# nipe1783/cudaSBMP

Measured on AMD Instinct MI355X. Metric: collision-checked samples/sec + time-to-first-solution, R2 car @1/2/4/8 GPUs, higher is better.
Workload: dtype f32; 1 GPU; c3: car, 262144 samples/iter/GPU, M=16777216, reference 5-box workspace, goal disabled, complete GNew clear; gnew_clear=complete, samples_per_iter_per_gpu=262144, maxTreeSize=16777216, numDisc=10, obstacles=5, seed=20240807, mean_frontier=1018, mean_accepted=1017, parallelism=single GPU

## Files before the change

cudasbmp_amd/_native.py:

```python
from __future__ import annotations

import ctypes
import os

_PKG = os.path.dirname(os.path.abspath(__file__))
LIB_PATH = os.path.join(_PKG, "libsbmp.so")

SBMP_OK = 0
SBMP_AGENT_CAR = 0
SBMP_AGENT_POINT = 1
SBMP_COMM_ID_BYTES = 128
SBMP_BATCH_REFERENCE = 0
SBMP_BATCH_FILL = 1


class NativeLibraryError(RuntimeError):
    pass


class SbmpError(RuntimeError):
    def __init__(self, status: int, func: str, msg: str):
        super().__init__(f"{func} failed with status {status}: {msg}")
        self.status = status

# ... 39 lines not shown


class ExpandBatchArgs(ctypes.Structure):
    _fields_ = [("count", ctypes.c_int), ("parents", ctypes.c_void_p), ("rng", ctypes.c_void_p),
                ("obstacles", ctypes.c_void_p), ("obstaclesCount", ctypes.c_int), ("agent", ctypes.c_int),
                ("numDisc", ctypes.c_int), ("agentLength", ctypes.c_float), ("width", ctypes.c_float),
                ("height", ctypes.c_float), ("N", ctypes.c_int), ("n", ctypes.c_int), ("R1Score", ctypes.c_void_p),
                ("R2Avail", ctypes.c_void_p), ("children", ctypes.c_void_p), ("valid", ctypes.c_void_p),
                ("r1", ctypes.c_void_p), ("r2", ctypes.c_void_p), ("accept", ctypes.c_void_p)]


class InsertBatchArgs(ctypes.Structure):
    _fields_ = [("slots", ctypes.c_int), ("gnew", ctypes.c_void_p), ("unexplored", ctypes.c_void_p),
                ("uParent", ctypes.c_void_p), ("samples", ctypes.c_void_p), ("parent", ctypes.c_void_p),
                ("costs", ctypes.c_void_p), ("treeSize", ctypes.c_int), ("maxTreeSize", ctypes.c_int),
                ("goalX", ctypes.c_float), ("goalY", ctypes.c_float), ("goalThreshold", ctypes.c_float),
                ("fixGNewClear", ctypes.c_int), ("inserted", ctypes.c_void_p), ("goalIndex", ctypes.c_void_p)]


class PathInfo(ctypes.Structure):
    _fields_ = [(n, ctypes.c_int) for n in ("stepForm", "obstacleForm", "residentGroups", "neededGroups", "exchange",
                                            "nranks", "rank", "commRanks", "listMirror",
                                            "fusedExchange", "oneshotCheck", "mirrorCheck", "fusedCheck", "rowTableLds",
                                            "rcpDivisions")]


class BatchInfo(ctypes.Structure):
    _fields_ = [(n, ctypes.c_int) for n in ("count", "groupsPerMember", "residentGroups", "membersPerLaunch",
                                            "launchesPerIteration", "batched")]


class GoalQuery(ctypes.Structure):
    _fields_ = [("x", ctypes.c_float), ("y", ctypes.c_float), ("radius", ctypes.c_float)]


class GoalAnswer(ctypes.Structure):
    _fields_ = [("count", ctypes.c_int), ("firstRow", ctypes.c_int), ("bestRow", ctypes.c_int),
                ("bestCost", ctypes.c_float), ("nearestRow", ctypes.c_int), ("nearestDistance", ctypes.c_float)]


class TreeRecheck(ctypes.Structure):
    _fields_ = [(n, ctypes.c_int) for n in ("rows", "alive", "blocked", "stale", "orphan", "cut", "firstDead")]


class TreeRecheckArgs(ctypes.Structure):
    _fields_ = [("state", ctypes.c_void_p), ("ctrl", ctypes.c_void_p), ("parent", ctypes.c_void_p),
                ("rows", ctypes.c_int), ("depthBound", ctypes.c_int), ("agent", ctypes.c_int),
# ... 157 lines not shown
```

cudasbmp_amd/csrc/kgmt_batch.cpp:

```cpp
#include <algorithm>
#include <cstdlib>
#include <cstring>

#include "kgmt_planner.h"

namespace sbmp {

template <typename F>
static auto for_member(int i, F f) {
    try {
        return f();
    } catch (const Error& e) {
        throw Error(e.status, "member " + std::to_string(i) + ": " + e.what());
    }
}

int BatchGroup::pack(const int* groupsPerMember, int count, int residentGroups, int* launchOfMember) {
    int launches = 0, used = 0;
    bool open = false;
    for (int i = 0; i < count; ++i) {
        const int g = groupsPerMember[i];
        if (g > residentGroups) {
            launchOfMember[i] = -1;
            open = false;
// ... 60 lines not shown
    for (int m = 0; m < B; ++m) members_[m]->begin(initials + 7 * m, goals + 7 * m, d_obstacles, nObs, seeds[m]);
    bool step = true;
    for (KgmtPlanner* k : members_) step = step && k->d_.stepMode && k->d_.hostPoll;
    for (KgmtPlanner* k : members_)
        if ((k->d_.stepMode != 0) != (members_[0]->d_.stepMode != 0))
            throw Error(SBMP_ERR_STATE, "batch members chose different forms");
    residentGroups_ = 0;
    membersPerLaunch_ = 1;
    std::fill(launchOf_.begin(), launchOf_.end(), -1);
    int nLaunches = 0;
    if (step) {
        KgmtPlanner& k0 = *members_[0];
        residentGroups_ = step_batch_resident_groups(k0.d_, k0.p_.agent, k0.expandVariant_);
        if (const char* v = getenv("SBMP_BATCH_MAX_GROUPS")) {
            const int cap = atoi(v);
            if (cap >= 0 && cap < residentGroups_) residentGroups_ = cap;
        }
        std::vector<int> groups(B);
        for (int m = 0; m < B; ++m) groups[m] = 1 + members_[m]->d_.nBlocks;
        nLaunches = pack(groups.data(), B, residentGroups_, launchOf_.data());
        if (nLaunches == 0 || std::count(launchOf_.begin(), launchOf_.end(), -1) > 0) {
            for (KgmtPlanner* k : members_) {
                k->d_.stepMode = 0;
                k->flushed_ = true;
                launch_finish(k->d_, 0, 0, stream_, k->timing(KgmtPlanner::K_FINISH));
            }
            SBMP_HIP(hipGetLastError());
            step = false;
            nLaunches = 0;
        }
    }
    batched_ = step;
    bool same = (int)launches_.size() == nLaunches;
    if (same) {
        std::vector<int> cnt(nLaunches, 0);
        for (int m = 0; m < B && batched_; ++m) cnt[launchOf_[m]]++;
        for (int l = 0; l < nLaunches; ++l) same = same && launches_[l].members == cnt[l];
    }
    if (!same) {
        SBMP_HIP(hipStreamSynchronize(stream_));
        free_launches();
        launches_.resize(nLaunches);
        for (int m = 0; m < B && batched_; ++m) {
            Launch& l = launches_[launchOf_[m]];
            if (l.members == 0) l.first = m;
            l.members++;
// ... 29 lines not shown
        launch_step_batch(k0.d_, t, expand, k0.p_.agent, k0.expandVariant_, l.dTable, l.members, l.maxGroups, stream_,
                          expand ? timer_.take(0, members_[0]->p_.profileKernels != 0) : KernelTiming());
    }
}

void BatchGroup::stage_member(KgmtPlanner* k, int t) {
    if (k->d_.stepMode) {
        k->stage_step(t);
    } else {
        k->stage_expand(t);
        k->stage_finish(t);
    }
}

void BatchGroup::enqueue(int iterations) {
    if (!begun_) throw Error(SBMP_ERR_STATE, "begin() has not been called");
    for (int i = 0; i < iterations; ++i) {
        int t = 0;
        for (KgmtPlanner* k : members_) t = k->take_iteration();
        if (t == 0) break;
        if (batched_) {
            for (KgmtPlanner* k : members_) k->upload_dev();
            issue(t, 1);
            for (KgmtPlanner* k : members_) k->flushed_ = false;
        } else {
            for (KgmtPlanner* k : members_) stage_member(k, t);
        }
        for (KgmtPlanner* k : members_) k->stage_fold(t);
    }
    SBMP_HIP(hipGetLastError());
}

void BatchGroup::flush() {
    if (!begun_) return;
    if (batched_) {
        bool any = false;
        for (KgmtPlanner* k : members_) any = any || !k->flushed_;
        if (!any) return;
        for (KgmtPlanner* k : members_) k->upload_dev();
        issue(members_[0]->t_next_, 0);
        for (KgmtPlanner* k : members_) k->flushed_ = true;
    } else {
        for (KgmtPlanner* k : members_) k->flush();
    }
}

void BatchGroup::sync() {
// ... 58 lines not shown
```

cudasbmp_amd/csrc/kgmt_device.h:

```cpp
#pragma once

#include <hip/hip_runtime.h>
#include <stdint.h>

#include <type_traits>

#include "sbmp/collision.h"
#include "sbmp/grid.h"
#include "sbmp/obstacle_grid.h"
#include "sbmp/sbmp_math.h"
#include "sbmp/xorwow.h"

#if defined(__clang__)
#pragma clang fp contract(off)
#endif

namespace sbmp {

constexpr int kBlock = 256;
constexpr int kWave = 64;
constexpr int kNoGoal = 0x7fffffff;
constexpr int kN = 16;
constexpr int kMaxR1 = kN * kN;
constexpr int kMaxR2Words = 2048;
// ... 44 lines not shown
constexpr int kNewReps = 8;
constexpr int kMaxStepBlocks = 1024;
constexpr int kNoGoalIdx = 0x7fffffff;
constexpr int kFastDivMax = 1 << 24;
constexpr int kStepEntry = 3;
constexpr int kPlannerInsertMax = 1024;
static_assert(kBlock / kWave == 4 && kMaxR1 == kBlock, "the flush and prefix code assumes 4 waves and 256 R1 cells");
constexpr int kInsertBase = 8;
constexpr int kRecordF4 = 3;

constexpr int kFxReplicas = 8;
constexpr int kFxShards = 8;
constexpr int kFxCounters = kFxReplicas * kFxShards;
constexpr int kFxStride = 32;
struct OneshotCompact {
    int nR1, rowOff, rowWords, cntOff, owned, nBlocks, newOff, newWords;
    int c16Off;
    int cR, cB, cN, total;
};

struct KgmtDev {
    int M, nSlots, nWords, nBlocks, numIterations, numDisc, N, n, nR1, nR2, nObs, cap, fixGNewClear;
    int batchRule;
    int nranks, rank;
    float width, height, agentLength, invAgentLength, goalThreshold, R1Size, R2Size, goalX, goalY;
    float rcpR1Size, rcpR2Size, rcpNumDisc, rcpAgentLength;
    float reachStep;
    float4* treeState;
    float4* treeCtrl;
    int* treeParent;
    float4* uState;
    float4* uCtrl;
    uint4* rngA;
    uint2* rngB;
    unsigned long long* gnewOut;
    unsigned long long* gnewIn;
    int* blockCountOut;
    const int* blockCountIn;
    int* pfxOut;
    const int* pfxIn;
    int* totOut;
    const int* totIn;
    unsigned long long* deltaOut;
    const unsigned long long* deltaIn;
    uint8_t* r2newOut;
    const uint8_t* r2newIn;
// ... 740 lines not shown
```

cudasbmp_amd/csrc/kgmt_kernels.hip:

```cpp
#include <hip/hip_ext.h>
#include <hip/hip_runtime.h>

#include "kgmt_device.h"
#include "kgmt_launch.h"
#include "kgmt_rules.h"

#if defined(__clang__)
#pragma clang fp contract(off)
#endif

namespace sbmp {

__device__ __forceinline__ int div_small(int a, int b) {
    int q = (int)((float)a * __builtin_amdgcn_rcpf((float)b));
    int r = a - q * b;
    if (r < 0) { --q; r += b; }
    if (r < 0) { --q; r += b; }
    if (r >= b) { ++q; r -= b; }
    if (r >= b) { ++q; }
    return q;
}

__device__ __forceinline__ int slot_div(const KgmtDev& d, int slot, int k) {
    if (k == 32) return slot >> 5;
// ... 1712 lines not shown
    int k = depth - 1;
    for (int j = node; j >= 0; j = d.treeParent[j], --k) {
        const float4 st = d.treeState[j];
        const float4 c = d.treeCtrl[j];
        rows[k] = j;
        float* o = samples + (size_t)k * 7;
        o[0] = st.x; o[1] = st.y; o[2] = st.z; o[3] = st.w;
        o[4] = c.x; o[5] = c.y; o[6] = c.z;
        costs[k] = c.w;
    }
}

__global__ void k_export_unexplored(KgmtDev d, float* samples, int* uParent) {
    for (int i = blockIdx.x * blockDim.x + threadIdx.x; i < d.nSlots; i += gridDim.x * blockDim.x) {
        const float4 s = d.uState[i];
        const float4 c = d.uCtrl[i];
        float* o = samples + (size_t)i * 7;
        o[0] = s.x; o[1] = s.y; o[2] = s.z; o[3] = s.w;
        o[4] = c.x; o[5] = c.y; o[6] = c.z;
        uParent[i] = __float_as_int(c.w);
    }
}

template <typename K, typename... Args>
static void launch(K kernel, dim3 grid, dim3 block, size_t shm, hipStream_t s, const KernelTiming& tm,
                   Args... args) {
    if (tm.start)
        hipExtLaunchKernelGGL(kernel, grid, block, (uint32_t)shm, s, tm.start, tm.stop, 0u, args...);
    else
        hipLaunchKernelGGL(kernel, grid, block, shm, s, args...);
}

int obstacle_form(const KgmtDev& d, int variant) {
    return with_obs_form(d, variant, [](auto obs) { return obs.value >= kObsReg ? kObsReg : obs.value; });
}

static size_t obs_lds_bytes(const KgmtDev& d, int obs) {
    return (obs == kObsLds || obs == kObsLds4) ? sizeof(float4) * (size_t)d.nObs : 0;
}

void launch_expand(const KgmtDev& d, int t, int agent, int blocks, int variant, hipStream_t s,
                   const KernelTiming& tm) {
    const dim3 grid(blocks), block(kBlock);
    with_obs_form(d, variant, [&](auto obs) {
        const size_t shm = obs_lds_bytes(d, obs.value);
        if (agent == 0) launch(k_expand<0, obs.value>, grid, block, shm, s, tm, d, t);
// ... 176 lines not shown

void launch_delay(double microseconds, hipStream_t s) {
    const long long ticks = (long long)(microseconds * 100.0);
    hipLaunchKernelGGL(k_delay, dim3(1), dim3(64), 0, s, ticks);
}

void launch_seed_root(const KgmtDev& d, float4 rs, float4 rc, int r1, int r2, hipStream_t s) {
    hipLaunchKernelGGL(k_seed_root, dim3(1), dim3(64), 0, s, d, rs, rc, r1, r2);
}

void launch_export_tree(const KgmtDev& d, float* samples, float* costs, hipStream_t s) {
    hipLaunchKernelGGL(k_export_tree, dim3(1024), dim3(256), 0, s, d, samples, costs);
}

void launch_solution_path(const KgmtDev& d, int node, int maxDepth, int* out, int* rows, float* samples, float* costs,
                          hipStream_t s) {
    hipLaunchKernelGGL(k_solution_path, dim3(1), dim3(64), 0, s, d, node, maxDepth, out, rows, samples, costs);
}

void launch_export_unexplored(const KgmtDev& d, float* samples, int* uParent, hipStream_t s) {
    hipLaunchKernelGGL(k_export_unexplored, dim3(1024), dim3(256), 0, s, d, samples, uParent);
}

}
```

cudasbmp_amd/csrc/kgmt_launch.h:

```cpp
#pragma once

#include <hip/hip_runtime.h>
#include <stdint.h>

#include <type_traits>
#include <vector>

#include "kgmt_device.h"

namespace sbmp {

struct KernelTiming {
    hipEvent_t start = nullptr;
    hipEvent_t stop = nullptr;
};

int obstacle_form(const KgmtDev& d, int variant);
template <int OBS>
using ObsForm = std::integral_constant<int, OBS>;

template <typename F>
auto with_obs_form(const KgmtDev& d, int variant, F f) {
    if (d.gridStart) return f(ObsForm<kObsGrid>{});
    if (d.nObs > kMaxLdsObs) return f(ObsForm<kObsGlobal>{});
// ... 56 lines not shown
    int rowOff, rows;
    int cntOff, owned, nBlocks;
    int newOff, newWords;
    int c16Off;
};
OneshotCompact oneshot_compact(const OneshotLayout& l);
void launch_oneshot(unsigned long long* const* inbox, const unsigned long long* send, unsigned long long* recv,
                    long long n, int nranks, int rank, unsigned long long seq, int* error, hipStream_t s,
                    const KernelTiming& tm = KernelTiming(), const OneshotLayout* compact = nullptr,
                    long long* tl = nullptr);
void launch_xsum(const unsigned long long* const* send, unsigned long long* const* recv, int nranks, long long n,
                 hipStream_t s);
void launch_delay(double microseconds, hipStream_t s);
void launch_fill_i32(int* p, int v, long long n, hipStream_t s);
void launch_fill_f32(float* p, float v, long long n, hipStream_t s);
void launch_init_slots(const KgmtDev& d, const Xorwow& base, const uint32_t* jumps, int nbits, int blocks,
                       hipStream_t s);
void launch_solution_path(const KgmtDev& d, int node, int maxDepth, int* out, int* rows, float* samples, float* costs,
                          hipStream_t s);
void launch_seed_root(const KgmtDev& d, float4 rs, float4 rc, int r1, int r2, hipStream_t s);
void launch_export_tree(const KgmtDev& d, float* samples, float* costs, hipStream_t s);
void launch_state_hash(const KgmtDev& d, int rows, int tp, int iters, unsigned long long* out, hipStream_t s);
void launch_export_unexplored(const KgmtDev& d, float* samples, int* uParent, hipStream_t s);

struct QueryAcc {
    unsigned long long best;
    unsigned long long nearest;
    unsigned count;
    unsigned first;
};
constexpr int kQueryTile = 16;
void launch_tree_query(const float4* state, const float4* ctrl, long long rows, const float* goalsXYT, int count,
                       QueryAcc* acc, hipStream_t s);

Xorwow curand_seed_state(uint64_t seed);
const std::vector<uint32_t>& subsequence_jump_matrices(int nbits);

}
```

cudasbmp_amd/csrc/kgmt_planner.cpp:

```cpp
#include "kgmt_planner.h"

#include <algorithm>
#include <chrono>
#include <climits>
#include <cmath>
#include <cstdio>
#include <cstring>
#include <fstream>
#include <iomanip>
#include <mutex>
#include <string>
#include <unordered_map>
#include <sys/stat.h>

#include "kgmt_launch.h"
#include "obstacle_grid.h"
#include "tree_pass.h"

namespace sbmp {

double now_ms() {
    using namespace std::chrono;
    return duration<double, std::milli>(steady_clock::now().time_since_epoch()).count();
}
// ... 27 lines not shown
        for (uint32_t m = 0; m < (1u << 23); ++m) {
            float a;
            const uint32_t bits = 0x3f800000u | m;
            std::memcpy(&a, &bits, 4);
            const volatile float ref = a / vb;
            const volatile float q0 = a * y;
            const float r = std::fma(-q0, b, a);
            const float q = std::fma(r, y, (float)q0);
            if (q != ref) {
                y = 0.0f;
                break;
            }
        }
    }
    std::lock_guard<std::mutex> g(mu);
    cache[key] = y;
    return y;
}

[[noreturn]] void throw_wait_error(int e) {
    if (e == kErrExchange)
        throw Error(SBMP_ERR_COMM, "k_oneshot: a peer rank's exchange flag did not arrive within 20 s");
    if (e == kErrStepHandoff)
        throw Error(SBMP_ERR_HIP, "k_step: the planner workgroup's hand-off did not arrive within 1 s");
    throw Error(SBMP_ERR_HIP, "in-kernel wait failed (status " + std::to_string(e) + ")");
}

static int round_up(long long x, long long m) { return (int)(((x + m - 1) / m) * m); }

KgmtPlanner::KgmtPlanner(const sbmp_kgmt_params& p, int nranks, int rank, Exchange* ex, hipStream_t shared)
    : p_(p), ex_(ex) {
    if (p.N * p.N != kMaxR1) throw Error(SBMP_ERR_INVALID_ARGUMENT, "N must be 16 (reference KGMT.cu:8 NUM_R1)");
    if (p.n < 1 || p.n > 16) throw Error(SBMP_ERR_INVALID_ARGUMENT, "n must be in [1, 16]");
    if (p.maxTreeSize < 1) throw Error(SBMP_ERR_INVALID_ARGUMENT, "maxTreeSize must be >= 1");
    if (p.numDisc < 1) throw Error(SBMP_ERR_INVALID_ARGUMENT, "numDisc must be >= 1");
    if (p.numIterations < 0) throw Error(SBMP_ERR_INVALID_ARGUMENT, "numIterations must be >= 0");
    if (p.samplesPerIteration < 0) throw Error(SBMP_ERR_INVALID_ARGUMENT, "samplesPerIteration must be >= 0");
    if (p.batchRule != SBMP_BATCH_REFERENCE && p.batchRule != SBMP_BATCH_FILL)
        throw Error(SBMP_ERR_INVALID_ARGUMENT, "unknown batchRule");
    if (p.batchRule == SBMP_BATCH_FILL && p.samplesPerIteration <= 0)
        throw Error(SBMP_ERR_INVALID_ARGUMENT, "batchRule FILL needs samplesPerIteration > 0");
    if (p.agent != SBMP_AGENT_CAR && p.agent != SBMP_AGENT_POINT) throw Error(SBMP_ERR_INVALID_ARGUMENT, "unknown agent");
    if (!(p.width > 0.0f) || !(p.height > 0.0f)) throw Error(SBMP_ERR_INVALID_ARGUMENT, "width/height must be > 0");
    if (nranks < 1 || nranks > kMaxRanks || rank < 0 || rank >= nranks)
        throw Error(SBMP_ERR_INVALID_ARGUMENT, "bad rank/nranks (at most 8 ranks)");
    int ndev = 0;
    SBMP_HIP(hipGetDeviceCount(&ndev));
    if (p.device < 0 || p.device >= ndev) throw Error(SBMP_ERR_INVALID_ARGUMENT, "no such HIP device");
// ... 116 lines not shown
                d.r2newIn = r2;
            }
        };
        views(xSend_, true);
        views(xRecv_, false);
    }
    d.sharded = nranks > 1 || ex != nullptr;
    {
        const char* v = getenv("SBMP_STEP");
        stepCapable_ = (!d.sharded && d.nBlocks <= kMaxStepBlocks && !(v && atoi(v) == 0)) || shStep_;
    }
    d.stepMode = stepCapable_ ? 1 : 0;
    d.stepCnt = nullptr;
    d.stepPub = nullptr;
    d.stepList = nullptr;
    d.stepDelta = nullptr;
    d.stepR2New = nullptr;
    if (stepCapable_) {
        d.stepPub = alloc<unsigned long long>((size_t)2 * (d.nR1 + d.nR2 / 32));
        if (!d.sharded) {
            d.stepCnt = alloc<int>((size_t)2 * kMaxStepBlocks);
            d.stepList = alloc<float4>((size_t)2 * d.nBlocks * kBlock * kStepEntry);
            d.stepDelta = alloc<unsigned long long>((size_t)3 * kDeltaReps * d.nR1);
            d.stepR2New = alloc<uint32_t>((size_t)3 * kNewReps * (d.nR2 / 32));
        }
        dDev_ = alloc<KgmtDev>(1);
        SBMP_HIP(hipHostMalloc(reinterpret_cast<void**>(&dStage_), sizeof(KgmtDev), hipHostMallocDefault));
    }
    d.devSelf = dDev_;
    d.recCap = expandBlocks_ * kBlock;
    d.recOut = d.sharded ? alloc<float4>((size_t)2 * kRecordF4 * d.recCap) : nullptr;
    for (int q = 0; q < kMaxRanks; ++q) d.recPeer[q] = nullptr;
    d.recPeer[rank] = d.recOut;
    d.logSlots = expandBlocks_ * kBlock;
    d.r2log = (d.nR2 <= kLogMaxR2) ? alloc<uint16_t>((size_t)kFoldEvery * d.logSlots) : nullptr;
    d.ctrl = alloc<IterCtrl>(p.numIterations + 2);
    d.status = alloc<PlannerStatus>(1);
    SBMP_HIP(hipHostMalloc(reinterpret_cast<void**>(&poll_), sizeof(PollBuf), hipHostMallocDefault));
    poll_->word = 0;
    d.hostPoll = nullptr;
    if (!d.sharded) SBMP_HIP(hipHostGetDevicePointer(reinterpret_cast<void**>(&d.hostPoll), &poll_->word, 0));
    d.timeline = nullptr;
    d.timelineFin = nullptr;
    d.timelineIter = -1;
    if (const char* v = getenv("SBMP_TIMELINE_ITER")) {
#ifndef SBMP_TIMELINE
        fprintf(stderr, "sbmp: SBMP_TIMELINE_ITER set, but k_step stamps only in a build with "
                        "SBMP_HIPCC_FLAGS=-DSBMP_TIMELINE (tools/_tl.sh); its expanding waves' stamps stay 0\n");
// ... 271 lines not shown
        if (obs_) SBMP_HIP(hipFree(obs_));
        obs_ = nullptr;
        SBMP_HIP(hipMalloc(&obs_, sizeof(float4) * nObs));
        obsCap_ = nObs;
    }
    if (nObs > 0)
        SBMP_HIP(hipMemcpyAsync(obs_, d_obstacles, sizeof(float4) * nObs, hipMemcpyDeviceToDevice, s));
    d.obstacles = obs_;
    d.nObs = nObs;
    d.obsNaN = 0;
    if (nObs > 0 && nObs <= kMaxRegObs) {
        float h[4 * kMaxRegObs];
        SBMP_HIP(hipMemcpyAsync(h, d_obstacles, sizeof(float) * 4 * nObs, hipMemcpyDeviceToHost, s));
        SBMP_HIP(hipStreamSynchronize(s));
        for (int i = 0; i < 4 * nObs; ++i)
            if (std::isnan(h[i])) d.obsNaN = 1;
    }
    d.gridG = 0;
    d.gridInvW = d.gridInvH = 0.0f;
    d.gridStart = nullptr;
    d.gridBoxes = nullptr;
    if (nObs > 0 && ((nObs > kMaxLdsObs && expandVariant_ != 5) || expandVariant_ == 4)) build_grid(d_obstacles, nObs);
    choose_form(d_obstacles, nObs);
    d.goalX = goal[0];
    d.goalY = goal[1];

    const int r1 = getR1(initial[0], initial[1], d.R1Size, d.N);
    const int r2 = getR2(initial[0], initial[1], r1, d.R1Size, d.N, d.R2Size, d.n);
    launch_seed_root(d, make_float4(initial[0], initial[1], initial[2], initial[3]),
                     make_float4(initial[4], initial[5], initial[6], 0.0f), r1, r2, s);
    launch_init_slots(d, curand_seed_state(seed), jumps_, nbits_, expandBlocks_, s);
    SBMP_HIP(hipGetLastError());
    if (const char* inj = getenv("SBMP_INJECT_WAIT_ERROR")) {
        const int code = atoi(inj);
        SBMP_HIP(hipStreamSynchronize(s));
        SBMP_HIP(hipMemcpy(&d.status->error, &code, sizeof(int), hipMemcpyHostToDevice));
    }

    t_next_ = 1;
    lastFolded_ = 0;
    aliveRows_ = -1;
    begun_ = true;
    wallMs_ = 0.0;
    wallFixed_ = false;
    SBMP_HIP(hipStreamSynchronize(s));
    poll_->word = 0;
// ... 54 lines not shown
    }
}

void KgmtPlanner::path_info(sbmp_path_info* out) {
    const KgmtDev& d = d_;
    out->stepForm = d.stepMode ? 1 : 0;
    const int form = obstacle_form(d, expandVariant_);
    out->obstacleForm = form == kObsGrid     ? SBMP_OBS_GRID
                        : form == kObsGlobal ? SBMP_OBS_GLOBAL
                        : form == kObsReg    ? SBMP_OBS_REGISTERS
                                             : SBMP_OBS_LDS;
    out->residentGroups = residentGroups_;
    out->neededGroups = neededGroups_;
    out->exchange = !d.sharded ? SBMP_EXCHANGE_NONE : (oneshot_ ? SBMP_EXCHANGE_ONESHOT : SBMP_EXCHANGE_COLLECTIVE);
    out->nranks = d.nranks;
    out->rank = d.rank;
    out->commRanks = ex_ ? ex_->comm_ranks() : 0;
    out->listMirror = d.stepMirror ? 1 : 0;
    out->fusedExchange = d.fusedX ? 1 : 0;
    out->oneshotCheck = oneshotCheck_;
    out->mirrorCheck = mirrorCheck_;
    out->fusedCheck = fusedCheck_;
    out->rowTableLds = d.c16Lds;
    out->rcpDivisions = (d.rcpR1Size != 0.0f ? SBMP_RCP_R1SIZE : 0) | (d.rcpR2Size != 0.0f ? SBMP_RCP_R2SIZE : 0) |
                        (d.rcpNumDisc != 0.0f ? SBMP_RCP_NUMDISC : 0) | (d.rcpAgentLength != 0.0f ? SBMP_RCP_AGENTLENGTH : 0);
}

void KgmtPlanner::build_grid(const float* d_obstacles, int nObs) {
    KgmtDev& d = d_;
    SBMP_HIP(hipStreamSynchronize(stream_));
    {
        std::vector<float> h((size_t)4 * nObs);
        SBMP_HIP(hipMemcpy(h.data(), d_obstacles, sizeof(float) * h.size(), hipMemcpyDeviceToHost));
        const HostObstacleGrid g =
            build_obstacle_grid(h.data(), nObs, d.width, d.height, std::min(grid_resolution(nObs), kMaxLdsGridG));
        const size_t nStart = g.start.size(), nBoxes = g.boxes.size() + kGridBatch;
        if (nStart > gridStartCap_) {
            if (gridStart_) SBMP_HIP(hipFree(gridStart_));
            gridStart_ = nullptr;
            SBMP_HIP(hipMalloc(&gridStart_, sizeof(int) * nStart));
            gridStartCap_ = nStart;
        }
        if (nBoxes > gridBoxesCap_) {
            if (gridBoxes_) SBMP_HIP(hipFree(gridBoxes_));
            gridBoxes_ = nullptr;
            SBMP_HIP(hipMalloc(&gridBoxes_, sizeof(float4) * nBoxes));
// ... 33 lines not shown
        stage_finish(t);
        stage_fold(t);
    }
    SBMP_HIP(hipGetLastError());
}

int KgmtPlanner::take_iteration() {
    if (!begun_ || t_next_ > p_.numIterations) return 0;
    return t_next_++;
}

void KgmtPlanner::stage_expand(int t) {
    launch_expand(d_, t, p_.agent, expandBlocks_, expandVariant_, stream_, timing(K_EXPAND));
}

void KgmtPlanner::stage_pack(int t) {
    launch_pack(d_, t, expandBlocks_, stream_, timing(K_PACK));
}

void KgmtPlanner::stage_step(int t) {
    upload_dev();
    launch_step(d_, t, 1, p_.agent, expandVariant_, stream_, timing(K_STEP));
    flushed_ = false;
}

void KgmtPlanner::stage_exchange(int t) {
    if (!ex_) return;
    if (d_.fusedX) {
        ++xSeq_;
        if (xSeq_ != d_.xSeqBase + (unsigned long long)t)
            throw Error(SBMP_ERR_STATE, "fused exchange: sequence " + std::to_string(xSeq_) + " at iteration " +
                                            std::to_string(t));
        return;
    }
    const unsigned long long* send = exchange_send(t);
    if (oneshot_) {
        ++xSeq_;
        OneshotLayout cx{};
        if (shStep_ && compactX_) {
            cx.on = 1;
            cx.nR1 = d_.nR1;
            cx.rowOff = d_.xRowOff;
            cx.rows = expandBlocks_;
            cx.cntOff = d_.xCntOff;
            cx.owned = expandBlocks_;
            cx.nBlocks = d_.nBlocks;
// ... 355 lines not shown
    SBMP_HIP(hipMalloc(&dI, sizeof(int) * (1 + (size_t)maxDepth)));
    SBMP_HIP(hipMalloc(&dF, sizeof(float) * 8 * (size_t)maxDepth));
    launch_solution_path(d_, node, maxDepth, dI, dI + 1, dF, dF + 7 * (size_t)maxDepth, stream_);
    std::vector<int> hi(1 + (size_t)maxDepth);
    std::vector<float> hf(8 * (size_t)maxDepth);
    SBMP_HIP(hipMemcpyAsync(hi.data(), dI, sizeof(int) * hi.size(), hipMemcpyDeviceToHost, stream_));
    SBMP_HIP(hipMemcpyAsync(hf.data(), dF, sizeof(float) * hf.size(), hipMemcpyDeviceToHost, stream_));
    SBMP_HIP(hipStreamSynchronize(stream_));
    (void)hipFree(dI);
    (void)hipFree(dF);
    const int len = hi[0];
    if (len < 0) throw Error(SBMP_ERR_STATE, "parent chain longer than numIterations + 2 rows");
    if ((rows || samples || costs) && capacity < len)
        throw Error(SBMP_ERR_INVALID_ARGUMENT, "capacity " + std::to_string(capacity) + " < path length " +
                                                   std::to_string(len));
    if (rows) memcpy(rows, hi.data() + 1, sizeof(int) * len);
    if (samples) memcpy(samples, hf.data(), sizeof(float) * 7 * len);
    if (costs) memcpy(costs, hf.data() + 7 * (size_t)maxDepth, sizeof(float) * len);
    return len;
}

void KgmtPlanner::copy_unexplored(float* samples, int* uParent) {
    sync();
    const size_t M = d_.M, n = d_.nSlots;
    float* dS = nullptr;
    int* dP = nullptr;
    SBMP_HIP(hipMalloc(&dS, sizeof(float) * n * 7));
    SBMP_HIP(hipMalloc(&dP, sizeof(int) * n));
    launch_export_unexplored(d_, dS, dP, stream_);
    std::vector<float> hs(n * 7);
    std::vector<int> hp(n);
    SBMP_HIP(hipMemcpyAsync(hs.data(), dS, sizeof(float) * n * 7, hipMemcpyDeviceToHost, stream_));
    SBMP_HIP(hipMemcpyAsync(hp.data(), dP, sizeof(int) * n, hipMemcpyDeviceToHost, stream_));
    SBMP_HIP(hipStreamSynchronize(stream_));
    (void)hipFree(dS);
    (void)hipFree(dP);
    if (d_.nranks > 1) {
        for (size_t i = 0; i < n; ++i) {
            if ((int)((i / kBlock) % d_.nranks) != d_.rank) {
                for (int q = 0; q < 7; ++q) hs[i * 7 + q] = 0.0f;
                hp[i] = -1;
            }
        }
    }
    if (samples) {
        memcpy(samples, hs.data(), sizeof(float) * n * 7);
// ... 250 lines not shown
```

cudasbmp_amd/csrc/kgmt_planner.h:

```cpp
#pragma once

#include <hip/hip_runtime.h>

#include <functional>
#include <stdexcept>
#include <string>
#include <vector>

#include "kgmt_device.h"
#include "kgmt_launch.h"
#include "sbmp/sbmp.h"

namespace sbmp {

struct Error : std::runtime_error {
    sbmp_status status;
    Error(sbmp_status s, const std::string& m) : std::runtime_error(m), status(s) {}
};

#define SBMP_HIP(expr)                                                                                   \
    do {                                                                                                 \
        hipError_t e_ = (expr);                                                                          \
        if (e_ != hipSuccess)                                                                            \
            throw ::sbmp::Error(SBMP_ERR_HIP, std::string(#expr) + ": " + hipGetErrorString(e_));      \
// ... 209 lines not shown

    sbmp_kgmt_params p_;
    KgmtDev d_{};
    KgmtDev* dDev_ = nullptr;
    KgmtDev* dStage_ = nullptr;
    bool uploaded_ = false;
    void upload_dev();
    hipStream_t stream_ = nullptr;
    bool ownStream_ = true;
    Exchange* ex_ = nullptr;
    int t_next_ = 1;
    bool begun_ = false;
    int slotsPadded_ = 0, expandBlocks_ = 0, nbits_ = 1;
    int expandVariant_ = 0;
    bool timelineDumped_ = false;
    struct PollBuf {
        IterCtrl ctrl;
        PlannerStatus status;
        unsigned long long word;
    };
    PollBuf* poll_ = nullptr;
    bool wallFixed_ = false;
    bool flushed_ = true;
    int lastFolded_ = 0;
    unsigned long long* local_ = nullptr;
    size_t localWords_ = 0;
    unsigned long long* xSend_ = nullptr;
    unsigned long long* xSendOdd_ = nullptr;
    bool shStep_ = false;
    bool stepCapable_ = false;
    int residentGroups_ = 0, neededGroups_ = 0;
    bool formLogged_ = false;
    void choose_form(const float* d_obstacles, int nObs);
    void build_grid(const float* d_obstacles, int nObs);
    unsigned long long* xRecv_ = nullptr;
    size_t xWords_ = 0;
    bool oneshot_ = false;
    bool oneshot_self_test();
    bool mirror_self_test();
    bool fused_self_test();
    int oneshotCheck_ = 0, mirrorCheck_ = 0, fusedCheck_ = 0;
    unsigned long long* inbox_[kMaxRanks] = {nullptr};
    bool compactX_ = true;
    unsigned long long xSeq_ = 0;
    uint32_t* jumps_ = nullptr;
    float4* obs_ = nullptr;
// ... 139 lines not shown
```

cudasbmp_amd/csrc/kgmt_step_body.h:

```cpp
    const int t = tx & 0x7fffffff, expand = (int)((unsigned)tx >> 31);
    const KgmtDev& d = *dp;
    const ShardView sv{SH ? (shRR >> 8) : 1, SH ? (shRR & 0xff) : 0, SH ? shRows : 0, G(shBw)};
    extern __shared__ float4 sDyn[];
    __shared__ int sR1P[kMaxR1];
    __shared__ StepPlan sPlan;
    __shared__ int sWaveCnt[kBlock / kWave];
    __shared__ int sWaveGoal[kBlock / kWave];
    __shared__ int sRed[2][kBlock / kWave];
    __shared__ float sPart[8];
    __shared__ int sCovInc[kMaxR1];

    constexpr bool kLdsObs = (OBS == kObsLds || OBS == kObsLds4);
    constexpr int kRegObs = obs_in_registers(OBS);
    int* const sPfx = reinterpret_cast<int*>(sDyn + (kLdsObs ? d.nObs : 0));
    uint32_t* const sNew = reinterpret_cast<uint32_t*>(sPfx + (SH ? sv.nRows : d.nBlocks) + 1);
    uint16_t* const sC16 = reinterpret_cast<uint16_t*>(sPfx + ((((SH ? sv.nRows : d.nBlocks) + 1 + (d.nR2 >> 5)) + 3) & ~3));
    if (blockIdx.x == 0) {
        step_planner<SH>(d, sv, t, expand, sPfx, sRed, sCovInc, sPart, sC16);
        if constexpr (SH) {
            if (expand && d.fusedX) step_planner_arrive(d, t);
        }
        return;
    }
    float4* const sObs = sDyn;
// ... 292 lines not shown
    int q1 = -1, q2 = -1;
    if (act) bins_k(out.state.x, out.state.y, d, &q1, &q2);
#if SBMP_VALU_DUP == 4
    if (act) {
        float x2 = out.state.x, y2 = out.state.y;
        asm volatile("" : "+v"(x2), "+v"(y2));
        int a2, b2;
        bins_k(x2, y2, d, &a2, &b2);
        asm volatile("" ::"v"(a2), "v"(b2));
    }
#endif
    const bool look = act && valid && q2 >= 0;
    unsigned long long sw = 0ull, aw = 0ull;
    if (look) {
        sw = __hip_atomic_load(pubCur + q1, __ATOMIC_RELAXED, __HIP_MEMORY_SCOPE_WORKGROUP);
        aw = __hip_atomic_load(pubCur + d.nR1 + (q2 >> 5), __ATOMIC_RELAXED, __HIP_MEMORY_SCOPE_WORKGROUP);
    }
    float u = 0.0f;
    if (valid) u = xorwow_uniform(rs);
    float4 cs = out.state;
    float4 cc = make_float4(out.a, out.steer, out.dur, __int_as_float(parent));
    float cost = parentCost + out.dur;
    if (act) {
        store_wt(d.uState, slot, cs);
        store_wt(d.uCtrl, slot, cc);
        store_wt(d.rngA, slot, make_uint4(rs.v0, rs.v1, rs.v2, rs.v3));
        store_wt(d.rngB, slot, make_uint2(rs.v4, rs.d));
        if (q1 >= 0) atomicAdd(&sR1P[q1], valid ? 1 : 0x10000);
        if (d.r2log) {
            store_wt(d.r2log, (t % kFoldEvery) * d.logSlots + b * kBlock + tid, r2_key(q2, valid));
        } else if (q2 >= 0) {
            __hip_atomic_fetch_add(G(valid ? d.R2Valid : d.R2Invalid) + q2, 1, __ATOMIC_RELAXED,
                                   __HIP_MEMORY_SCOPE_AGENT);
        }
    }
    {
        const unsigned want = (unsigned)t;
        bool stale = look && (((unsigned)(sw >> 32) != want) | ((unsigned)(aw >> 32) != want));
        if (__ballot(stale) != 0ull) {
            const long long t0 = (long long)__builtin_amdgcn_s_memrealtime();
            for (;;) {
                __builtin_amdgcn_s_sleep(8);
                if (stale) {
                    sw = __hip_atomic_load(pubCur + q1, __ATOMIC_RELAXED, __HIP_MEMORY_SCOPE_AGENT);
                    aw = __hip_atomic_load(pubCur + d.nR1 + (q2 >> 5), __ATOMIC_RELAXED, __HIP_MEMORY_SCOPE_AGENT);
                    stale = ((unsigned)(sw >> 32) != want) | ((unsigned)(aw >> 32) != want);
                }
// ... 139 lines not shown
```

cudasbmp_amd/kgmt.py:

```python
from __future__ import annotations

import ctypes
import time
from typing import Optional

import numpy as np

from . import _native as nat

AGENTS = {"car": nat.SBMP_AGENT_CAR, "point": nat.SBMP_AGENT_POINT}
BATCH_RULES = {"reference": nat.SBMP_BATCH_REFERENCE, "fill": nat.SBMP_BATCH_FILL}


def reference_seed_from_time(t: Optional[float] = None) -> int:
    v = ctypes.c_int(int(time.time() if t is None else t)).value
    return v & 0xFFFFFFFFFFFFFFFF


class DeviceBuffer:

    def __init__(self, host: np.ndarray):
        host = np.ascontiguousarray(host, dtype=np.float32).ravel()
        p = ctypes.c_void_p()
        nat.call("sbmp_device_upload_f32", host.ctypes.data_as(ctypes.c_void_p), host.size, ctypes.byref(p))
# ... 332 lines not shown
        nat.call("sbmp_kgmt_kernel_stats", self._h, ctypes.cast(arr, ctypes.c_void_p), 16, ctypes.byref(cnt))
        return {arr[i].name.decode(): (arr[i].launches, arr[i].totalMs) for i in range(min(cnt.value, 16))}

    def reset_kernel_stats(self) -> None:
        nat.call("sbmp_kgmt_reset_kernel_stats", self._h)

    OBSTACLE_FORMS = ("registers", "lds", "grid", "global")
    EXCHANGES = ("none", "oneshot", "collective")
    RCP_DIVISORS = (("R1Size", 1), ("R2Size", 2), ("numDisc", 4), ("agentLength", 8))

    def path_info(self) -> dict:
        pi = nat.PathInfo()
        nat.call("sbmp_kgmt_path_info", self._h, ctypes.byref(pi))
        return {"form": "k_step" if pi.stepForm else "two-launch",
                "obstacle_form": self.OBSTACLE_FORMS[pi.obstacleForm] if 0 <= pi.obstacleForm < 4 else pi.obstacleForm,
                "resident_groups": pi.residentGroups, "needed_groups": pi.neededGroups,
                "exchange": self.EXCHANGES[pi.exchange] if 0 <= pi.exchange < 3 else pi.exchange,
                "nranks": pi.nranks, "rank": pi.rank, "rccl_nranks": pi.commRanks,
                "list_mirror": bool(pi.listMirror), "fused_exchange": bool(pi.fusedExchange),
                "oneshot_check": {0: "not run", 1: "passed", -1: "failed"}.get(pi.oneshotCheck, pi.oneshotCheck),
                "mirror_check": {0: "not run", 1: "passed", -1: "failed"}.get(pi.mirrorCheck, pi.mirrorCheck),
                "fused_check": {0: "not run", 1: "passed", -1: "failed"}.get(pi.fusedCheck, pi.fusedCheck),
                "row_table_lds": bool(pi.rowTableLds),
                "rcp_divisions": {k: bool(pi.rcpDivisions & b) for k, b in self.RCP_DIVISORS}}

    def kernel_samples(self, name: str) -> np.ndarray:
        cnt = ctypes.c_int()
        nat.call("sbmp_kgmt_kernel_samples", self._h, name.encode(), None, 0, ctypes.byref(cnt))
        out = np.zeros(max(1, cnt.value), dtype=np.float32)
        nat.call("sbmp_kgmt_kernel_samples", self._h, name.encode(), out.ctypes.data_as(ctypes.c_void_p),
                 cnt.value, ctypes.byref(cnt))
        return out[: cnt.value]

    def enqueue_delay(self, microseconds: float) -> None:
        nat.call("sbmp_kgmt_enqueue_delay", self._h, float(microseconds))

    def set_profiling(self, enabled: bool) -> None:
        nat.call("sbmp_kgmt_set_profiling", self._h, int(bool(enabled)))

    def state_hash(self) -> int:
        h = ctypes.c_uint64()
        nat.call("sbmp_kgmt_state_hash", self._h, ctypes.byref(h))
        return int(h.value)
```

include/sbmp/sbmp.h:

```cpp
#ifndef SBMP_H
#define SBMP_H

#include <stddef.h>
#include <stdint.h>

#ifdef __cplusplus
extern "C" {
#endif

#define SBMP_ABI_VERSION 1

typedef int sbmp_status;
#define SBMP_OK 0
#define SBMP_ERR_INVALID_ARGUMENT 1
#define SBMP_ERR_HIP 2
#define SBMP_ERR_IO 3
#define SBMP_ERR_OUT_OF_MEMORY 4
#define SBMP_ERR_STATE 5
#define SBMP_ERR_UNSUPPORTED 6
#define SBMP_ERR_COMM 7

#define SBMP_AGENT_CAR 0
#define SBMP_AGENT_POINT 1

// ... 41 lines not shown

#define SBMP_OBS_REGISTERS 0
#define SBMP_OBS_LDS 1
#define SBMP_OBS_GRID 2
#define SBMP_OBS_GLOBAL 3
#define SBMP_EXCHANGE_NONE 0
#define SBMP_EXCHANGE_ONESHOT 1
#define SBMP_EXCHANGE_COLLECTIVE 2
typedef struct sbmp_path_info {
    int stepForm;
    int obstacleForm;
    int residentGroups;
    int neededGroups;
    int exchange;
    int nranks, rank;
    int commRanks;
    int listMirror;
    int fusedExchange;
    int oneshotCheck;
    int mirrorCheck;
    int fusedCheck;
    int rowTableLds;
    int rcpDivisions;
} sbmp_path_info;
#define SBMP_RCP_R1SIZE 1
#define SBMP_RCP_R2SIZE 2
#define SBMP_RCP_NUMDISC 4
#define SBMP_RCP_AGENTLENGTH 8

typedef struct sbmp_kgmt sbmp_kgmt;

int sbmp_abi_version(void);
const char* sbmp_status_string(sbmp_status s);
const char* sbmp_last_error(void);

sbmp_status sbmp_kgmt_default_params(sbmp_kgmt_params* p);

typedef struct sbmp_system_config {
    sbmp_kgmt_params params;
    float initial[7];
    float goal[7];
    char obstacles[1024];
} sbmp_system_config;
sbmp_status sbmp_load_system_config(const char* path, sbmp_system_config* out);

sbmp_status sbmp_kgmt_create(const sbmp_kgmt_params* p, sbmp_kgmt** out);
// ... 218 lines not shown
```

Before: 23.59 billion samples/s.

## Defer child state stores in k_step, rematerialise lazily on export

```diff
diff --git a/cudasbmp_amd/_native.py b/cudasbmp_amd/_native.py
--- a/cudasbmp_amd/_native.py
+++ b/cudasbmp_amd/_native.py
@@ -85,7 +85,7 @@
     _fields_ = [(n, ctypes.c_int) for n in ("stepForm", "obstacleForm", "residentGroups", "neededGroups", "exchange",
                                             "nranks", "rank", "commRanks", "listMirror",
                                             "fusedExchange", "oneshotCheck", "mirrorCheck", "fusedCheck", "rowTableLds",
-                                            "rcpDivisions")]
+                                            "rcpDivisions", "lazyChildren")]
 
 
 class BatchInfo(ctypes.Structure):
diff --git a/cudasbmp_amd/csrc/kgmt_batch.cpp b/cudasbmp_amd/csrc/kgmt_batch.cpp
--- a/cudasbmp_amd/csrc/kgmt_batch.cpp
+++ b/cudasbmp_amd/csrc/kgmt_batch.cpp
@@ -106,6 +106,7 @@
         if (nLaunches == 0 || std::count(launchOf_.begin(), launchOf_.end(), -1) > 0) {
             for (KgmtPlanner* k : members_) {
                 k->d_.stepMode = 0;
+                k->d_.lazyChildren = 0;
                 k->flushed_ = true;
                 launch_finish(k->d_, 0, 0, stream_, k->timing(KgmtPlanner::K_FINISH));
             }
@@ -181,7 +182,10 @@
         if (batched_) {
             for (KgmtPlanner* k : members_) k->upload_dev();
             issue(t, 1);
-            for (KgmtPlanner* k : members_) k->flushed_ = false;
+            for (KgmtPlanner* k : members_) {
+                k->flushed_ = false;
+                k->childrenStale_ = k->d_.lazyChildren != 0;
+            }
         } else {
             for (KgmtPlanner* k : members_) stage_member(k, t);
         }
diff --git a/cudasbmp_amd/csrc/kgmt_device.h b/cudasbmp_amd/csrc/kgmt_device.h
--- a/cudasbmp_amd/csrc/kgmt_device.h
+++ b/cudasbmp_amd/csrc/kgmt_device.h
@@ -90,6 +90,7 @@
 struct KgmtDev {
     int M, nSlots, nWords, nBlocks, numIterations, numDisc, N, n, nR1, nR2, nObs, cap, fixGNewClear;
     int batchRule;
+    int lazyChildren;
     int nranks, rank;
     float width, height, agentLength, invAgentLength, goalThreshold, R1Size, R2Size, goalX, goalY;
     float rcpR1Size, rcpR2Size, rcpNumDisc, rcpAgentLength;
diff --git a/cudasbmp_amd/csrc/kgmt_kernels.hip b/cudasbmp_amd/csrc/kgmt_kernels.hip
--- a/cudasbmp_amd/csrc/kgmt_kernels.hip
+++ b/cudasbmp_amd/csrc/kgmt_kernels.hip
@@ -1758,6 +1758,47 @@
     }
 }
 
+template <int AGENT, int OBS>
+__global__ __launch_bounds__(kBlock) void k_materialise_children(KgmtDev d) {
+    extern __shared__ float4 sObs[];
+    constexpr bool kLdsObs = (OBS == kObsLds || OBS == kObsLds4);
+    constexpr int kRegObs = obs_in_registers(OBS);
+    const int tid = threadIdx.x;
+    const int lane = tid & (kWave - 1);
+    const int slot = (int)blockIdx.x * kBlock + tid;
+    float4 ro[kRegObs > 0 ? kRegObs : 1];
+#pragma unroll
+    for (int i = 0; i < kRegObs; ++i) ro[i] = d.obstacles[i];
+    float4 cc = make_float4(0.0f, 0.0f, 0.0f, __int_as_float(-1));
+    if (slot < d.nSlots) cc = d.uCtrl[slot];
+    const int parent = __float_as_int(cc.w);
+    const bool act = parent >= 0 && parent < d.M;
+    const float4 p = d.treeState[act ? parent : 0];
+    if (kLdsObs) {
+        for (int i = tid; i < d.nObs; i += kBlock) sObs[i] = d.obstacles[i];
+        __syncthreads();
+    }
+    const float4* obs = (kRegObs > 0) ? ro : kLdsObs ? sObs : d.obstacles;
+    const ChildCtl ctl = stored_controls<AGENT>(cc, d);
+    ChildOut out;
+    bool fast = false;
+    if constexpr (AGENT == 0 && kRegObs > 0) {
+        fast = car_fast_ok(d);
+        if (fast) {
+            const float4 oLane = G(d.obstacles)[lane % kRegObs];
+            (void)car_propagate_fast<OBS>(p, 2 * lane, act, ctl, d, obs, oLane, out);
+        }
+    }
+    if (!fast) {
+        out = ChildOut{};
+        if (act) {
+            if (AGENT == 0) (void)car_euler<OBS>(p, ctl, d, obs, out);
+            else (void)point_euler<OBS>(p, ctl, d, obs, out);
+        }
+    }
+    if (act) d.uState[slot] = out.state;
+}
+
 template <typename K, typename... Args>
 static void launch(K kernel, dim3 grid, dim3 block, size_t shm, hipStream_t s, const KernelTiming& tm,
                    Args... args) {
@@ -1980,4 +2021,13 @@
     hipLaunchKernelGGL(k_export_unexplored, dim3(1024), dim3(256), 0, s, d, samples, uParent);
 }
 
-}
+void launch_materialise_children(const KgmtDev& d, int agent, int variant, hipStream_t s) {
+    const dim3 grid(d.nBlocks), block(kBlock);
+    with_obs_form(d, variant, [&](auto obs) {
+        const size_t shm = obs_lds_bytes(d, obs.value);
+        if (agent == 0) launch(k_materialise_children<0, obs.value>, grid, block, shm, s, KernelTiming(), d);
+        else launch(k_materialise_children<1, obs.value>, grid, block, shm, s, KernelTiming(), d);
+    });
+}
+
+}
diff --git a/cudasbmp_amd/csrc/kgmt_launch.h b/cudasbmp_amd/csrc/kgmt_launch.h
--- a/cudasbmp_amd/csrc/kgmt_launch.h
+++ b/cudasbmp_amd/csrc/kgmt_launch.h
@@ -102,6 +102,7 @@
 void launch_export_tree(const KgmtDev& d, float* samples, float* costs, hipStream_t s);
 void launch_state_hash(const KgmtDev& d, int rows, int tp, int iters, unsigned long long* out, hipStream_t s);
 void launch_export_unexplored(const KgmtDev& d, float* samples, int* uParent, hipStream_t s);
+void launch_materialise_children(const KgmtDev& d, int agent, int variant, hipStream_t s);
 
 struct QueryAcc {
     unsigned long long best;
diff --git a/cudasbmp_amd/csrc/kgmt_planner.cpp b/cudasbmp_amd/csrc/kgmt_planner.cpp
--- a/cudasbmp_amd/csrc/kgmt_planner.cpp
+++ b/cudasbmp_amd/csrc/kgmt_planner.cpp
@@ -73,8 +73,7 @@
     if (e == kErrExchange)
         throw Error(SBMP_ERR_COMM, "k_oneshot: a peer rank's exchange flag did not arrive within 20 s");
     if (e == kErrStepHandoff)
-        throw Error(SBMP_ERR_HIP, "k_step: the planner workgroup's hand-off did not arrive within 1 s");
-    throw Error(SBMP_ERR_HIP, "in-kernel wait failed (status " + std::to_string(e) + ")");
+        throw Error(SBMP_ERR_HIP, "k_step: the planner workgroup's hand-off did not arrive within 1 s");    throw Error(SBMP_ERR_HIP, "in-kernel wait failed (status " + std::to_string(e) + ")");
 }
 
 static int round_up(long long x, long long m) { return (int)(((x + m - 1) / m) * m); }
@@ -237,8 +236,7 @@
             d.stepCnt = alloc<int>((size_t)2 * kMaxStepBlocks);
             d.stepList = alloc<float4>((size_t)2 * d.nBlocks * kBlock * kStepEntry);
             d.stepDelta = alloc<unsigned long long>((size_t)3 * kDeltaReps * d.nR1);
-            d.stepR2New = alloc<uint32_t>((size_t)3 * kNewReps * (d.nR2 / 32));
-        }
+            d.stepR2New = alloc<uint32_t>((size_t)3 * kNewReps * (d.nR2 / 32));        }
         dDev_ = alloc<KgmtDev>(1);
         SBMP_HIP(hipHostMalloc(reinterpret_cast<void**>(&dStage_), sizeof(KgmtDev), hipHostMallocDefault));
     }
@@ -556,6 +554,11 @@
     d.gridBoxes = nullptr;
     if (nObs > 0 && ((nObs > kMaxLdsObs && expandVariant_ != 5) || expandVariant_ == 4)) build_grid(d_obstacles, nObs);
     choose_form(d_obstacles, nObs);
+    {
+        const char* lv = getenv("SBMP_LAZY_CHILDREN");
+        d.lazyChildren = (d.stepMode && !d.sharded && d.fixGNewClear && !(lv && atoi(lv) == 0)) ? 1 : 0;
+    }
+    childrenStale_ = false;
     d.goalX = goal[0];
     d.goalY = goal[1];
 
@@ -656,6 +659,7 @@
     out->mirrorCheck = mirrorCheck_;
     out->fusedCheck = fusedCheck_;
     out->rowTableLds = d.c16Lds;
+    out->lazyChildren = d.lazyChildren;
     out->rcpDivisions = (d.rcpR1Size != 0.0f ? SBMP_RCP_R1SIZE : 0) | (d.rcpR2Size != 0.0f ? SBMP_RCP_R2SIZE : 0) |
                         (d.rcpNumDisc != 0.0f ? SBMP_RCP_NUMDISC : 0) | (d.rcpAgentLength != 0.0f ? SBMP_RCP_AGENTLENGTH : 0);
 }
@@ -735,6 +739,14 @@
     upload_dev();
     launch_step(d_, t, 1, p_.agent, expandVariant_, stream_, timing(K_STEP));
     flushed_ = false;
+    childrenStale_ = d_.lazyChildren != 0;
+}
+
+void KgmtPlanner::materialise_children() {
+    if (!childrenStale_) return;
+    launch_materialise_children(d_, p_.agent, expandVariant_, stream_);
+    SBMP_HIP(hipGetLastError());
+    childrenStale_ = false;
 }
 
 void KgmtPlanner::stage_exchange(int t) {
@@ -1136,6 +1148,7 @@
 
 void KgmtPlanner::copy_unexplored(float* samples, int* uParent) {
     sync();
+    materialise_children();
     const size_t M = d_.M, n = d_.nSlots;
     float* dS = nullptr;
     int* dP = nullptr;
diff --git a/cudasbmp_amd/csrc/kgmt_planner.h b/cudasbmp_amd/csrc/kgmt_planner.h
--- a/cudasbmp_amd/csrc/kgmt_planner.h
+++ b/cudasbmp_amd/csrc/kgmt_planner.h
@@ -255,6 +255,8 @@
     PollBuf* poll_ = nullptr;
     bool wallFixed_ = false;
     bool flushed_ = true;
+    bool childrenStale_ = false;
+    void materialise_children();
     int lastFolded_ = 0;
     unsigned long long* local_ = nullptr;
     size_t localWords_ = 0;
diff --git a/cudasbmp_amd/csrc/kgmt_step_body.h b/cudasbmp_amd/csrc/kgmt_step_body.h
--- a/cudasbmp_amd/csrc/kgmt_step_body.h
+++ b/cudasbmp_amd/csrc/kgmt_step_body.h
@@ -338,7 +338,7 @@
     float4 cc = make_float4(out.a, out.steer, out.dur, __int_as_float(parent));
     float cost = parentCost + out.dur;
     if (act) {
-        store_wt(d.uState, slot, cs);
+        if (!d.lazyChildren) store_wt(d.uState, slot, cs);
         store_wt(d.uCtrl, slot, cc);
         store_wt(d.rngA, slot, make_uint4(rs.v0, rs.v1, rs.v2, rs.v3));
         store_wt(d.rngB, slot, make_uint2(rs.v4, rs.d));
diff --git a/cudasbmp_amd/kgmt.py b/cudasbmp_amd/kgmt.py
--- a/cudasbmp_amd/kgmt.py
+++ b/cudasbmp_amd/kgmt.py
@@ -378,7 +378,8 @@
                 "mirror_check": {0: "not run", 1: "passed", -1: "failed"}.get(pi.mirrorCheck, pi.mirrorCheck),
                 "fused_check": {0: "not run", 1: "passed", -1: "failed"}.get(pi.fusedCheck, pi.fusedCheck),
                 "row_table_lds": bool(pi.rowTableLds),
-                "rcp_divisions": {k: bool(pi.rcpDivisions & b) for k, b in self.RCP_DIVISORS}}
+                "rcp_divisions": {k: bool(pi.rcpDivisions & b) for k, b in self.RCP_DIVISORS},
+                "lazy_children": bool(pi.lazyChildren)}
 
     def kernel_samples(self, name: str) -> np.ndarray:
         cnt = ctypes.c_int()
diff --git a/include/sbmp/sbmp.h b/include/sbmp/sbmp.h
--- a/include/sbmp/sbmp.h
+++ b/include/sbmp/sbmp.h
@@ -87,6 +87,7 @@
     int fusedCheck;
     int rowTableLds;
     int rcpDivisions;
+    int lazyChildren;
 } sbmp_path_info;
 #define SBMP_RCP_R1SIZE 1
 #define SBMP_RCP_R2SIZE 2
```

Measured after the change: 23.88 billion samples/s, median of 6. 1.01x the previous value.
